# ma921/BASQ

Hardware: AMD Instinct MI355X
Metric: recombination batches/sec (N candidates -> n points) at N=1e6 d=10 (higher is better)
Workload: dtype f64

## Files before the change

basq_amd/_batch.py:

```python
from __future__ import annotations

import dataclasses
import time
import warnings

import torch

from . import _config as cfg
from . import _epochs
from ._basis import _mm_splitk, _ShardedProducts, _skip_test_matrix_draw, _Timer, make_cov_psd, nystrom_basis_steps
from ._lib import ROLE_A, ROLE_B
from ._partition import RoundGeometry, initial_shards
from ._plan import Plan, ReductionTimeout, _NoWait, _recorded_event, classes_for, late_split
from ._rounds_async import AsyncRounds
from ._rounds_sync import SyncRounds
from ._sums import FusedSums, OpaqueSums, exact_unit_plan


class Batch(AsyncRounds, SyncRounds):

    def __init__(self, ops, comm, pts_local, gid0: int, n_total: int, pts_nys, num_pts: int, kernel, trace=None,
                 variant: str = "basq", init_weights=None, objective=None, pipelined: bool = False, owner: int | None = None,
                 draw_on_owner: bool = False):
        if n_total >= 2 ** 31:
            raise ValueError("pool sizes >= 2^31 are not supported")
        self.ops, self.comm, self.trace = ops, comm, trace
        self.notes = []
        d = int(pts_nys.shape[1]) if pts_nys.dim() == 2 else 0
        if not getattr(kernel, "opaque", False) and not kernel.base.fits_packed_rows(d):
            from .kernels import CallableKernel

            self.notes.append(f"dimension {d} exceeds the fused kernels' packed-row limit ({kernel.base.__class__.__name__}: "
                              "d <= 38); the kernel is evaluated densely on the device (basq_dense_blocksum_f64 path)")
            kernel = CallableKernel(kernel)
        self.kernel, self.variant = kernel, variant
        self.pts_local_in, self.pts_nys_in = pts_local, pts_nys
        self.gid0, self.n_total, self.num_pts = int(gid0), int(n_total), int(num_pts)
        self.init_weights, self.objective = init_weights, objective
        self.pipelined = pipelined
        self.owner = None if (owner is None or comm.world == 1) else int(owner) % comm.world
        self.draw_on_owner = bool(draw_on_owner) and self.owner is not None
        m_nys = int(pts_nys.shape[0]) if pts_nys.dim() >= 1 else 0
        self.plan = Plan.of(kernel, variant, objective, comm, ops, trace, n_sets=2 * (min(int(num_pts) - 1, m_nys) + 1),
                            owner=self.owner)

    def steps(self):
        try:
            return (yield from self._steps())
        finally:
            self._release()

    def _release(self):
        sums = self.__dict__.get("sums")
        if sums is not None:
            sums.b = None
        keep = ("notes", "plan", "drew_test_matrix")
        for k in list(self.__dict__):
            if k not in keep:
                self.__dict__[k] = None

    def _steps(self):
        ops = self.ops
        if self.n_total == 0:
            dev = getattr(ops, "device", "cpu")
            return torch.empty(0, dtype=torch.int64, device=dev), torch.empty(0, dtype=torch.float64, device=dev)
        t_all = time.perf_counter()
        self._prepare_operands()
        self._init_candidates()
        pre, late = self._prelaunch_round1()
        t0 = time.perf_counter()
        U = yield from self._basis_steps(late)
        self._trace_phase("basis", t0)
        if self.trace is not None and self.trace.keep_tensors:
            self.trace.U = U.clone()
        self._extend_basis(U)
        self._trace_phase("setup", t0)
        if self.plan.async_rounds and self.R > self.S:
            if _epochs.eligible(self):
                outcome = yield from _epochs.async_rounds_columns(self, pre)
            else:
                outcome = yield from self._async_rounds(pre)
            pre = None
            if outcome == "basis":
                self._recover_basis()
                self._init_candidates()
            elif outcome:
                self.notes.append("descriptor-driven rounds hit a round that did not keep exactly half of the sets; the "
                                  "rounds were repeated one read-back at a time")
                self._init_candidates()
        if self._basis_bad is not None:
            flag, ready = ops.to_host_async(self._basis_bad, "basis_flag")
            yield ready
            if float(flag[0]) != 0.0:
                self._recover_basis()
            self._basis_bad = None
        idx, w = yield from self._sync_rounds(pre)
        self._trace_phase("total", t_all)
        for msg in self.notes:
            warnings.warn("basq_amd.recombination: " + msg, RuntimeWarning, stacklevel=3)
        return idx, w

    def _trace_phase(self, key, t0):
        if self.trace is not None:
            if self.trace.host_sync:
                self.ops.synchronize()
            self.trace.add_time(key, time.perf_counter() - t0)

    def _prepare_operands(self):
        ops, kernel, plan = self.ops, self.kernel, self.plan
        self.pts_nys = pts_nys = ops.to_device(self.pts_nys_in, torch.float64)
        self.pts_local = ops.to_device(self.pts_local_in, torch.float64)
        self.m, self.d = m, d = pts_nys.shape
        self.base = None if plan.opaque else kernel.base
        self.post = kernel.posterior if plan.posterior else None
        self.spec = None if plan.opaque else self.base.spec(d)
        if plan.posterior:
            self.spec = dataclasses.replace(self.spec, accurate_exp=True)
        self.kp = d if plan.opaque else ops.kp(d)
        self.kscale = 1.0 if plan.opaque else self.spec.outputscale
        self.center = None if plan.opaque else ops.col_mean(pts_nys)
# ... 26 lines not shown
            nys_cat = torch.cat(nys_rows, 0) if len(nys_rows) > 1 else pts_nys
            nys_ext = ops.pack(self.spec, nys_cat, self.center, ROLE_A, pad_rows_to=64)
            if nys_ext.shape[0] < ((self.m_ext + 63) // 64) * 64:
                nys_ext = torch.cat([nys_ext, ops.zeros(64, self.kp)], 0)
            if self.wrow:
                nys_ext[self.zero_row_idx].zero_()
            self.nys_ext = nys_ext
        self.exact_blocks = plan.opaque and kernel.resolve_mode(ops, pts_nys, self.S)
        self.sums = OpaqueSums(self) if plan.opaque else FusedSums(self)

    def _init_candidates(self):
        ops, comm, plan = self.ops, self.comm, self.plan
        pts_local = self.pts_local
        Rl = pts_local.shape[0]
        self.cand = (pts_local if Rl > 0 else ops.zeros(1, self.d)) if plan.opaque \
            else ops.pack(self.spec, pts_local, self.center, ROLE_B)
        self.mu, self.gid = ops.init_state(Rl, self.gid0, self.n_total)
        self.wx = None
        if plan.warp != "none":
            self.wx = self.kernel.mean(ops, pts_local, self.center) if Rl > 0 else ops.empty(1)
        self.off, self.R, self.Rl = self.gid0, self.n_total, Rl
        self.obj_full = self.obj_live = None
        if plan.objective:
            self.obj_full = self.obj_live = ops.to_device(self.objective, torch.float64).reshape(-1)
            if self.obj_full.shape[0] != Rl:
                raise ValueError("objective must have one entry per candidate")
        if plan.sober and self.init_weights is not None:
            w0 = ops.to_device(self.init_weights, torch.float64)
            if w0.shape[0] != Rl:
                raise ValueError("init_weights must have one entry per local candidate")
            nz = torch.nonzero(w0 != 0).reshape(-1)
            self.cand, self.mu, self.gid = self.cand[nz].contiguous(), w0[nz].contiguous(), self.gid[:Rl][nz].contiguous()
            if self.obj_live is not None:
                self.obj_live = self.obj_live[nz].contiguous()
            if self.wx is not None:
                self.wx = self.wx[nz].contiguous()
            Rl = int(nz.numel())
            counts = torch.tensor([float(Rl)], dtype=torch.float64, device=self.mu.device)
            if comm.world > 1:
                counts = comm.all_gather(counts).reshape(-1)
            counts = [int(v) for v in counts.cpu()]
            self.off, self.R, self.Rl = sum(counts[:comm.rank]), sum(counts), Rl
            if Rl == 0:
                self.cand, self.mu, self.gid = ops.zeros(1, self.kp), ops.zeros(1), ops.zeros(1, dtype=torch.int64)
        self.cls = None
        self.R_lo = self.R

    def _prelaunch_round1(self):
        if self.R > self.S and not self.plan.opaque:
            pre = self.sums.evaluate(RoundGeometry.of(self.R, self.S), self.S, defer_last=True)
            return pre, pre[5]
        return None, None

    def _basis_steps(self, late):
        ops, comm, kernel, trace = self.ops, self.comm, self.kernel, self.trace
        m, q, pts_nys = self.m, self.q, self.pts_nys
        self._basis_bad = self._basis_fallback = None
        self._basis_on_rank0 = False
        if cfg.SHARDED_BASIS and comm.world > 1 and not self.plan.sober and not self.plan.opaque:
            shards = initial_shards(m, comm.world)
            r0, mr = shards[comm.rank]
            with _Timer(ops, trace, "basis.gram"):
                A_rows = kernel.dense(ops, pts_nys[r0:r0 + mr].contiguous(), pts_nys, self.center, diag_offset=r0) \
                    if mr else ops.zeros(0, m)
            prod = _ShardedProducts(ops, comm, A_rows, shards, m, drawer=self.owner if self.draw_on_owner else 0,
                                    lockstep=not self.draw_on_owner)
            self.drew_test_matrix = comm.rank == prod.drawer or prod.lockstep
            res = yield from nystrom_basis_steps(ops, prod, self.num_pts - 1, trace, overlap=late, notes=self.notes)
            if res.bad is not None:
                self._basis_bad, self._basis_fallback = res.bad.to(torch.float64), res.fallback
            return res.U
        self._basis_on_rank0 = True
        bad = None
        if comm.rank == 0:
            with _Timer(ops, trace, "basis.gram"):
                A = kernel.dense(ops, pts_nys, pts_nys, self.center)
                if self.plan.sober:
                    A = make_cov_psd(A)
            res = yield from nystrom_basis_steps(ops, A, self.num_pts - 1, trace, overlap=late, notes=self.notes)
            del A
            U, bad, self._basis_fallback = res.U, res.bad, res.fallback
            assert U.shape[0] == q
        else:
            U = ops.empty(q, m)
            _skip_test_matrix_draw(ops, m, self.num_pts - 1)
            if late is not None:
                late()
            if cfg.BASIS_SVD and cfg.GPU_RANGE_FINDER and self.num_pts - 1 <= m:
                yield _recorded_event(ops)
        if comm.world > 1:
            buf = ops.empty(q + 1, m)
            if comm.rank == 0:
                buf[:q] = U
                buf[q].zero_()
                if bad is not None:
                    buf[q, 0:1] = bad.to(torch.float64)
            comm.broadcast(buf)
            U = buf[:q]
            self._basis_bad = buf[q, 0:1] if (cfg.GPU_RANGE_FINDER and not cfg.BASIS_SVD and self.num_pts - 1 <= m) else None
        elif bad is not None:
            self._basis_bad = bad.to(torch.float64)
        return U

    def _recover_basis(self):
        ops, comm = self.ops, self.comm
        if not self._basis_on_rank0:
            U = self._basis_fallback()
        else:
            U = self._basis_fallback() if comm.rank == 0 else ops.empty(self.q, self.m)
            if comm.world > 1:
                U = U.contiguous()
                comm.broadcast(U)
        if self.trace is not None and self.trace.keep_tensors:
            self.trace.U = U.clone()
        self._basis_bad = None
        self._extend_basis(U)

    def _extend_basis(self, U):
        ops, plan, q, m = self.ops, self.plan, self.q, self.m
        self.U = U
        Um = U
        if plan.warp != "none":
            mu_pt = self.kernel.mean(ops, self.pts_nys, self.center)
            Um = (U * mu_pt.unsqueeze(0)).contiguous()
        U_cols = [Um]
        self.bmatT = None
        if self.post is not None:
            W = ops.to_device(self.post.W, torch.float64)
            Bmat = _mm_splitk(ops, self.base.dense(ops, self.pts_nys, self.Xo, self.center), W, 1)
            U_cols.append(-_mm_splitk(ops, Um, Bmat, 8))
            if plan.warp == "wsabim":
                self.bmatT = ops.zeros(((self.n_obs + 3) // 4) * 4, ((m + 63) // 64) * 64)
                self.bmatT[:self.n_obs, :m] = Bmat.t()
        U_ext = torch.cat(U_cols, 1) if len(U_cols) > 1 else Um
# ... 7 lines not shown
```

basq_amd/_config.py:

```python
from __future__ import annotations

HOST_LAPACK_THREADS = 8
HOST_SVD_THREADS = 1

OWN_RANGE_GEMM = True
FUSED_CHOLQR = True
BASIS_SVD = False
GPU_RANGE_FINDER = True
GPU_NULLSPACE = True

REPLICATED_REDUCTION = True
OWNER_RANK_REDUCTION = True
SHARDED_CHOLQR = True
SHARDED_BASIS = True

LATE_CHUNKS = 0
LATE_CLASSES = 0
LATE_CLASSES_PIPELINED = 0

CLASS_SUMS = True
MAX_CLASSES = 16
IRR_COLUMNS = True
PIPELINED_SIDE_STREAM = False
ASYNC_ROUNDS = True

RAND_COPY_STREAM = True

SPIN_WAIT = False

PSD_EIG_MAX_M = 4096
```

basq_amd/_ops.py:

```python
from __future__ import annotations

import ctypes as C

import torch

from . import _lib
from ._lib import KernelSpecC, ROLE_A, ROLE_B, check


def _ptr(t):
    return C.c_void_p(t.data_ptr()) if t is not None else C.c_void_p(0)


_COPY_STREAMS = {}
_SIDE_OPS = {}
PROJECT_KSPLIT_MAX = 64


class HipOps:

    name = "hip"

    def __init__(self, device, stream=None):
        self.device = torch.device(device)
# ... 449 lines not shown
            W = torch.linalg.solve_triangular(torch.tril(G).t(), eye, upper=True)
            return torch.nan_to_num(W).contiguous(), info
        W = self.empty(q, q)
        check(self.lib.basq_chol_inv_f64(_ptr(G), q, _ptr(W), _ptr(info), float(rel_tol), self._stream()),
              "basq_chol_inv_f64")
        return W, info

    CHOL_FACTOR_MAX_Q = 200
    TRSM_MAX_Q = 318

    def chol_factor(self, G, rel_tol=1e-12):
        self._chk(G)
        info = self.empty(1, dtype=torch.int32)
        check(self.lib.basq_chol_factor_f64(_ptr(G), G.shape[0], _ptr(info), float(rel_tol), self._stream()),
              "basq_chol_factor_f64")
        return info

    def trsm_rows(self, X, L):
        self._chk(X)
        self._chk(L)
        rows, q = X.shape
        out = self.empty(rows, q)
        check(self.lib.basq_trsm_rows_f64(_ptr(X), q, rows, q, _ptr(L), _ptr(out), q, self._stream()), "basq_trsm_rows_f64")
        return out

    CHOLQR_FUSED_MAX_Q = 200

    def cholqr(self, G, X, rel_tol=1e-12):
        self._chk(G)
        self._chk(X)
        rows, q = X.shape
        out = self.empty(rows, q)
        info = self.empty(2, dtype=torch.int32)
        check(self.lib.basq_cholqr_f64(_ptr(G), q, _ptr(info), float(rel_tol), _ptr(X), q, rows, _ptr(out), q, self._stream()),
              "basq_cholqr_f64")
        return out, info[:1]

    def gemm(self, A, B, alpha=1.0):
        self._chk(A)
        self._chk(B)
        Mr, K = A.shape
        K2, N = B.shape
        assert K == K2
        Cm = self.empty(Mr, N)
        check(self.lib.basq_gemm_f64(_ptr(A), K, _ptr(B), N, _ptr(Cm), N, Mr, N, K, float(alpha), self._stream()),
              "basq_gemm_f64")
        return Cm

    def matmul(self, A, B):
        return torch.matmul(A, B)

    SKINNY_MAX_N = 208

    @staticmethod
    def _skinny_ksplit(M, K, N):
        rows_per_wave = 16 if N > 112 else 32
        row_waves = (M + rows_per_wave - 1) // rows_per_wave
        return max(1, min(round(1900 / row_waves), K // 160))

    def skinny_gemm(self, A, B, trans=False, ksplit=None):
        if A.dtype != torch.float64 or B.dtype != torch.float64 or A.stride(1) != 1 or B.stride(1) != 1:
            raise ValueError("expected float64 matrices with unit column stride")
        K, M = (A.shape[0], A.shape[1]) if trans else (A.shape[1], A.shape[0])
        N = B.shape[1]
        assert B.shape[0] == K and N <= self.SKINNY_MAX_N
        if ksplit is None:
            ksplit = self._skinny_ksplit(M, K, N)
        out = self.empty(M, N)
        work = self.empty(ksplit * M * N) if ksplit > 1 else None
        check(self.lib.basq_skinny_gemm_f64(_ptr(A), A.stride(0), 1 if trans else 0, M, K, _ptr(B), B.stride(0), N,
                                            int(ksplit), _ptr(work), _ptr(out), self._stream()), "basq_skinny_gemm_f64")
        return out

    PIN_CACHE_ENTRIES = 48

    def _pinned(self, shape, dtype, tag):
        cache = self.__dict__.setdefault("_pin_cache", {})
        key = (tag, tuple(shape), dtype)
        buf = cache.pop(key, None)
        if buf is None:
            buf = torch.empty(tuple(shape), dtype=dtype, pin_memory=True)
            while len(cache) >= self.PIN_CACHE_ENTRIES:
                cache.pop(next(iter(cache)))
        cache[key] = buf
        return buf

    def release_caches(self):
        for k in ("_pin_cache", "_ws_cache", "_ut_cache"):
            self.__dict__.pop(k, None)

    def to_host(self, t, tag="d2h"):
        buf = self._pinned(t.shape, t.dtype, tag)
        buf.copy_(t, non_blocking=True)
        self.torch_stream().synchronize()
        return buf

    def to_host_async(self, t, tag="d2h"):
        buf = self._pinned(t.shape, t.dtype, tag)
        buf.copy_(t, non_blocking=True)
        ev = torch.cuda.Event()
        ev.record(self.torch_stream())
        return buf, ev

    def host_uniform(self, n, tag):
        buf = self._pinned((n,), torch.float64, tag)
        return torch.rand(n, dtype=torch.float64, out=buf)

    def from_pinned(self, buf):
        return buf.to(self.device, non_blocking=True)

    def from_pinned_side(self, buf):
        side = _COPY_STREAMS.get(self.device.index)
        if side is None:
            side = _COPY_STREAMS[self.device.index] = torch.cuda.Stream(device=self.device)
        with torch.cuda.stream(side):
            t = buf.to(self.device, non_blocking=True)
            ev = torch.cuda.Event()
            ev.record(side)
        main = self.torch_stream()
        main.wait_event(ev)
        t.record_stream(main)
        return t

    def from_host(self, t, tag="h2d"):
        buf = self._pinned(t.shape, t.dtype, tag)
        buf.copy_(t)
        return buf.to(self.device, non_blocking=True)

    def synchronize(self):
        self.torch_stream().synchronize()

    def record_event(self, timing=True):
        ev = torch.cuda.Event(enable_timing=timing)
        ev.record(self.torch_stream())
        return ev

    def wait_event(self, ev):
        self.torch_stream().wait_event(ev)

    def side_ops(self):
        idx = self.device.index
        ops = _SIDE_OPS.get(idx)
        if ops is None:
            ops = _SIDE_OPS[idx] = HipOps(self.device, stream=torch.cuda.Stream(device=self.device))
        return ops

    def own_side_ops(self):
        ops = self.__dict__.get("_own_side")
        if ops is None:
            ops = self.__dict__["_own_side"] = HipOps(self.device, stream=torch.cuda.Stream(device=self.device))
        return ops

    def side_context(self):
        return torch.cuda.stream(self.side_ops().stream)

    def own_side_context(self):
        return torch.cuda.stream(self.own_side_ops().stream)
```

basq_amd/csrc/basq_linalg.hip:

```cpp
#include "basq_common.hpp"

template <int JT>
__global__ void __launch_bounds__(256) gemm_kernel(const double* __restrict__ A, long long lda, long long a_ks,
                                                   const double* __restrict__ B, long long ldb, long long bstride,
                                                   int nsum, double* __restrict__ C, long long ldc, long long cstride,
                                                   int M, int N, int K, int kslice, double alpha, int zdiv,
                                                   long long b_zstride) {
    const int lane = threadIdx.x & 63, wave = threadIdx.x >> 6;
    const int c = lane & 15, g = lane >> 4;
    const int r0 = blockIdx.x * (16 * JT);
    const int n0 = (blockIdx.y * 4 + wave) * 16;
    if (n0 >= N) return;
    B += (long long)(blockIdx.z / zdiv) * b_zstride;
    const int k0 = (blockIdx.z % zdiv) * kslice;
    int k1 = k0 + kslice;
    if (k1 > K) k1 = K;
    const int col = (n0 + c < N) ? (n0 + c) : (N - 1);
    long long arow[JT];
#pragma unroll
    for (int jt = 0; jt < JT; ++jt) {
        int r = r0 + jt * 16 + c;
        if (r >= M) r = M - 1;
        arow[jt] = (long long)r * lda;
    }
    d4 acc[JT];
#pragma unroll
    for (int jt = 0; jt < JT; ++jt) acc[jt] = (d4){0.0, 0.0, 0.0, 0.0};
    for (int k = k0; k < k1; k += 16) {
        double bv[4], av[4][JT];
#pragma unroll
        for (int u = 0; u < 4; ++u) {
            const int kg = k + 4 * u + g;
            const bool kin = kg < k1;
            double b = 0.0;
            if (kin) {
                const double* bp = B + (long long)kg * ldb + col;
                b = bp[0];
                for (int v = 1; v < nsum; ++v) b += bp[(long long)v * bstride];
            }
            bv[u] = b;
#pragma unroll
            for (int jt = 0; jt < JT; ++jt) av[u][jt] = kin ? A[arow[jt] + kg * a_ks] : 0.0;
        }
#pragma unroll
        for (int u = 0; u < 4; ++u)
#pragma unroll
            for (int jt = 0; jt < JT; ++jt)
                acc[jt] = __builtin_amdgcn_mfma_f64_16x16x4f64(av[u][jt], bv[u], acc[jt], 0, 0, 0);
    }
    if (n0 + c < N) {
        double* Cz = C + (long long)blockIdx.z * cstride;
#pragma unroll
        for (int jt = 0; jt < JT; ++jt)
#pragma unroll
            for (int r = 0; r < 4; ++r) {
                const int row = r0 + jt * 16 + g + 4 * r;
                if (row < M) Cz[(long long)row * ldc + n0 + c] = alpha * acc[jt][r];
            }
    }
}

template <int CTRL>
__device__ __forceinline__ double dpp_row_f64(double v) {
    const long long b = __double_as_longlong(v);
    const int lo = __builtin_amdgcn_mov_dpp((int)b, CTRL, 0xf, 0xf, true);
    const int hi = __builtin_amdgcn_mov_dpp((int)(b >> 32), CTRL, 0xf, 0xf, true);
    return __longlong_as_double(((long long)hi << 32) | (unsigned int)lo);
}

template <int NT, int REM, int JT, bool TRANS>
__global__ void __launch_bounds__(256) __attribute__((amdgpu_waves_per_eu(2)))
skinny_gemm_kernel(const double* __restrict__ A, long long lda, long long a_bstride, const double* __restrict__ B,
                   long long ldb, double* __restrict__ C, long long ldc, long long cstride, int M, int N, int K, int kslice,
                   int nz) {
    const int lane = threadIdx.x & 63, wave = threadIdx.x >> 6;
    const int c = lane & 15, g = lane >> 4;
    A += (long long)blockIdx.y * a_bstride;
    C += (long long)blockIdx.y * nz * cstride;
    const int zslice = blockIdx.x % nz;
    const int r0 = ((blockIdx.x / nz) * 4 + wave) * (16 * JT);
    const int k0 = zslice * kslice;
    int k1 = k0 + kslice;
    if (k1 > K) k1 = K;
    int rg[4];
    rg[0] = c >> 2;
    rg[1] = (__builtin_amdgcn_update_dpp(0, c, 0x124, 0xf, 0xf, false) & 15) >> 2;
    rg[2] = (__builtin_amdgcn_update_dpp(0, c, 0x128, 0xf, 0xf, false) & 15) >> 2;
    rg[3] = (__builtin_amdgcn_update_dpp(0, c, 0x12c, 0xf, 0xf, false) & 15) >> 2;
    long long aoff[JT];
#pragma unroll
    for (int jt = 0; jt < JT; ++jt) {
        int r = r0 + jt * 16 + c;
        if (r >= M) r = M - 1;
        aoff[jt] = TRANS ? (long long)r : (long long)r * lda;
    }
    constexpr int NB = NT + REM;
    constexpr int W = 16 * NT + 4 * REM;
    int bcol[NB];
#pragma unroll
    for (int nt = 0; nt < NT; ++nt) bcol[nt] = (nt * 16 + c < N) ? (nt * 16 + c) : (N - 1);
#pragma unroll
    for (int r = 0; r < REM; ++r) bcol[NT + r] = (16 * NT + 4 * r + (c & 3) < N) ? (16 * NT + 4 * r + (c & 3)) : (N - 1);
    double acc[JT][4][NT], accr[JT][REM > 0 ? REM : 1];
#pragma unroll
    for (int jt = 0; jt < JT; ++jt)
#pragma unroll
        for (int r = 0; r < (REM > 0 ? REM : 1); ++r) accr[jt][r] = 0.0;
#pragma unroll
    for (int jt = 0; jt < JT; ++jt)
#pragma unroll
        for (int rho = 0; rho < 4; ++rho)
#pragma unroll
            for (int nt = 0; nt < NT; ++nt) acc[jt][rho][nt] = 0.0;
    auto kidx = [&](int k, int u) { return TRANS ? (k + 4 * u + g) : (k + 4 * g + u); };
    const bool a_vec = !TRANS && ((lda & 1) == 0) && (((uintptr_t)A & 15) == 0);
    auto mfma_step = [&](const double (&a)[JT], const double (&bv)[NB]) {
#pragma unroll
        for (int jt = 0; jt < JT; ++jt) {
            double ar[4];
            ar[0] = a[jt];
            ar[1] = dpp_row_f64<0x124>(ar[0]);
            ar[2] = dpp_row_f64<0x128>(ar[0]);
            ar[3] = dpp_row_f64<0x12c>(ar[0]);
#pragma unroll
            for (int rho = 0; rho < 4; ++rho)
#pragma unroll
                for (int nt = 0; nt < NT; ++nt)
                    acc[jt][rho][nt] = __builtin_amdgcn_mfma_f64_4x4x4f64(ar[rho], bv[nt], acc[jt][rho][nt], 0, 0, 0);
#pragma unroll
            for (int r = 0; r < REM; ++r)
                accr[jt][r] = __builtin_amdgcn_mfma_f64_4x4x4f64(a[jt], bv[NT + r], accr[jt][r], 0, 0, 0);
        }
    };

    constexpr int NLD = (W + 15) / 16;
    __shared__ double btile[2][16][W];
    const int over_rows = (W + (int)ldb - 1) / (int)ldb;
    const int kfast_end = (k1 < K - over_rows) ? k1 : (K - over_rows);
    const int ktrips = (kfast_end > k0) ? (kfast_end - k0) / 16 : 0;
    int kdone = k0;
    if (ktrips > 0 && (TRANS || a_vec)) {
        const int skk = threadIdx.x >> 4, sc = threadIdx.x & 15;
        const char* bbase = reinterpret_cast<const char*>(B + (long long)k0 * ldb);
        const unsigned soff = (unsigned)(((long long)skk * ldb + sc) * 8);
        const long long btrip = 16 * ldb * 8;
        auto stage_load = [&](double (&sr)[NLD]) {
#pragma unroll
            for (int i = 0; i < NLD; ++i)
                if (16 * i + 16 <= W || sc + 16 * i < W) sr[i] = *reinterpret_cast<const double*>(bbase + soff + 128 * i);
        };
        auto stage_store = [&](int buf, const double (&sr)[NLD]) {
#pragma unroll
            for (int i = 0; i < NLD; ++i)
                if (16 * i + 16 <= W || sc + 16 * i < W) btile[buf][skk][sc + 16 * i] = sr[i];
        };
        auto lds_b = [&](int buf, int u, double (&bv)[NB]) {
            const int kk = TRANS ? (4 * u + g) : (4 * g + u);
#pragma unroll
            for (int nt = 0; nt < NT; ++nt) bv[nt] = btile[buf][kk][16 * nt + c];
#pragma unroll
            for (int r = 0; r < REM; ++r) bv[NT + r] = btile[buf][kk][16 * NT + 4 * r + (c & 3)];
        };
        const double* ap[JT];
#pragma unroll
        for (int jt = 0; jt < JT; ++jt) ap[jt] = TRANS ? (A + (long long)(k0 + g) * lda + aoff[jt]) : (A + aoff[jt] + k0 + 4 * g);
        const long long atrip = TRANS ? 16 * lda : 16;
        auto fetch_a = [&](double (&av)[4][JT]) {
#pragma unroll
            for (int jt = 0; jt < JT; ++jt) {
                if (TRANS) {
#pragma unroll
                    for (int u = 0; u < 4; ++u) av[u][jt] = ap[jt][(long long)(4 * u) * lda];
                } else {
                    const double2* p = reinterpret_cast<const double2*>(ap[jt]);
                    const double2 lo = p[0], hi = p[1];
                    av[0][jt] = lo.x;
                    av[1][jt] = lo.y;
                    av[2][jt] = hi.x;
                    av[3][jt] = hi.y;
                }
            }
        };
        double av[4][JT], bv[NB], sr[NLD];
        fetch_a(av);
        stage_load(sr);
        stage_store(0, sr);
        __syncthreads();
        lds_b(0, 0, bv);
        for (int t = 0; t < ktrips; ++t) {
            const bool last = (t + 1 == ktrips);
            const int buf = t & 1;
            if (!last) {
                bbase += btrip;
                stage_load(sr);
            }
            const long long ainc = last ? 0 : atrip;
#pragma unroll
            for (int jt = 0; jt < JT; ++jt) ap[jt] += ainc;
            double avn[4][JT];
            fetch_a(avn);
#pragma unroll
            for (int u = 0; u < 4; ++u) {
                double bvn[NB];
                if (u < 3) lds_b(buf, u + 1, bvn);
                mfma_step(av[u], bv);
                if (u < 3) {
#pragma unroll
                    for (int nt = 0; nt < NB; ++nt) bv[nt] = bvn[nt];
                }
            }
            if (!last) stage_store(buf ^ 1, sr);
            __syncthreads();
            if (!last) lds_b(buf ^ 1, 0, bv);
#pragma unroll
            for (int u = 0; u < 4; ++u)
#pragma unroll
                for (int jt = 0; jt < JT; ++jt) av[u][jt] = avn[u][jt];
        }
        kdone = k0 + 16 * ktrips;
    }
    for (int k = kdone; k < k1; k += 16) {
#pragma unroll
        for (int u = 0; u < 4; ++u) {
            const int kk = kidx(k, u);
            const int kc = (kk < k1) ? kk : (k1 - 1);
            double a[JT], bv[NB];
#pragma unroll
            for (int jt = 0; jt < JT; ++jt) {
                const double v = TRANS ? A[(long long)kc * lda + aoff[jt]] : A[aoff[jt] + kc];
                a[jt] = (kk < k1) ? v : 0.0;
            }
            const double* bp = B + (long long)kc * ldb;
#pragma unroll
            for (int nt = 0; nt < NB; ++nt) bv[nt] = bp[bcol[nt]];
            mfma_step(a, bv);
        }
    }
    double* Cz = C + (long long)zslice * cstride;
#pragma unroll
    for (int nt = 0; nt < NT; ++nt) {
        if (nt * 16 + c >= N) continue;
#pragma unroll
        for (int jt = 0; jt < JT; ++jt)
#pragma unroll
            for (int rho = 0; rho < 4; ++rho) {
                const int row = r0 + jt * 16 + 4 * rg[rho] + g;
                if (row < M) Cz[(long long)row * ldc + nt * 16 + c] = acc[jt][rho][nt];
            }
    }
#pragma unroll
    for (int r = 0; r < REM; ++r) {
        const int col = 16 * NT + 4 * r + (c & 3);
        if (col >= N) continue;
#pragma unroll
        for (int jt = 0; jt < JT; ++jt) {
            const int row = r0 + jt * 16 + 4 * (c >> 2) + g;
            if (row < M) Cz[(long long)row * ldc + col] = accr[jt][r];
        }
    }
}

template <int NT, int REM, int JT>
static void launch_skinny(bool trans, int M, int nz, int nbatch, hipStream_t st, const double* A, long long lda,
                          long long a_bstride, const double* B, long long ldb, double* C, long long ldc, long long cstride,
                          int N, int K, int kslice) {
    dim3 grid((unsigned)((M + 64 * JT - 1) / (64 * JT)) * (unsigned)nz, (unsigned)nbatch);
    if (trans)
        hipLaunchKernelGGL((skinny_gemm_kernel<NT, REM, JT, true>), grid, dim3(256), 0, st, A, lda, a_bstride, B, ldb, C, ldc,
                           cstride, M, N, K, kslice, nz);
    else
        hipLaunchKernelGGL((skinny_gemm_kernel<NT, REM, JT, false>), grid, dim3(256), 0, st, A, lda, a_bstride, B, ldb, C, ldc,
                           cstride, M, N, K, kslice, nz);
}

static void dispatch_skinny(bool trans, int M, int nz, int nbatch, hipStream_t st, const double* A, long long lda,
                            long long a_bstride, const double* B, long long ldb, double* C, long long cstride, int N, int K,
                            int kslice) {
    const int nt = (N + 15) / 16, ng = (N + 3) / 4;
    const bool small = (long long)((M + 127) / 128) * nz * nbatch <= 128;
    if (small && ng == 25) launch_skinny<6, 1, 1>(trans, M, nz, nbatch, st, A, lda, a_bstride, B, ldb, C, N, cstride, N, K, kslice);
    else if (small && nt <= 4) launch_skinny<4, 0, 1>(trans, M, nz, nbatch, st, A, lda, a_bstride, B, ldb, C, N, cstride, N, K, kslice);
    else if (small && nt <= 7) launch_skinny<7, 0, 1>(trans, M, nz, nbatch, st, A, lda, a_bstride, B, ldb, C, N, cstride, N, K, kslice);
    else if (ng == 25) launch_skinny<6, 1, 2>(trans, M, nz, nbatch, st, A, lda, a_bstride, B, ldb, C, N, cstride, N, K, kslice);
    else if (ng == 50) launch_skinny<12, 2, 1>(trans, M, nz, nbatch, st, A, lda, a_bstride, B, ldb, C, N, cstride, N, K, kslice);
    else if (nt <= 4) launch_skinny<4, 0, 2>(trans, M, nz, nbatch, st, A, lda, a_bstride, B, ldb, C, N, cstride, N, K, kslice);
    else if (nt <= 7) launch_skinny<7, 0, 2>(trans, M, nz, nbatch, st, A, lda, a_bstride, B, ldb, C, N, cstride, N, K, kslice);
    else launch_skinny<13, 0, 1>(trans, M, nz, nbatch, st, A, lda, a_bstride, B, ldb, C, N, cstride, N, K, kslice);
}

__global__ void chunk_sum_kernel(const double* __restrict__ Xpart, long long n, int n_chunks, double* __restrict__ Xsum) {
    const long long e = ((long long)blockIdx.x * blockDim.x + threadIdx.x) * 2;
    if (e + 1 < n) {
        double2 v = *reinterpret_cast<const double2*>(Xpart + e);
        for (int c = 1; c < n_chunks; ++c) {
            const double2 u = *reinterpret_cast<const double2*>(Xpart + (long long)c * n + e);
            v.x += u.x;
            v.y += u.y;
        }
        *reinterpret_cast<double2*>(Xsum + e) = v;
    } else if (e < n) {
        double v = Xpart[e];
        for (int c = 1; c < n_chunks; ++c) v += Xpart[(long long)c * n + e];
        Xsum[e] = v;
    }
}

__device__ __forceinline__ double ordered_strided_sum(const double* __restrict__ p, int n, long long stride) {
    double v = 0.0;
    int z = 0;
    for (; z + 8 <= n; z += 8) {
        double t[8];
#pragma unroll
        for (int u = 0; u < 8; ++u) t[u] = p[(long long)(z + u) * stride];
#pragma unroll
        for (int u = 0; u < 8; ++u) v += t[u];
    }
    for (; z < n; ++z) v += p[(long long)z * stride];
    return v;
}

__global__ void project_reduce_kernel(const double* __restrict__ work, int ksplit, int q, int S,
                                      const double* __restrict__ totpart, int n_chunks, double* __restrict__ out) {
    const int idx = blockIdx.x * blockDim.x + threadIdx.x;
    if (idx >= (q + 1) * S) return;
    const int r = idx / S, s = idx % S;
    double v = 0.0;
    if (r == 0) {
        for (int cc = 0; cc < n_chunks; ++cc) v += totpart[(long long)cc * S + s];
    } else {
        v = ordered_strided_sum(work + (long long)(r - 1) * S + s, ksplit, (long long)q * S);
    }
    out[idx] = v;
}

__global__ void finalize_kernel(const double* __restrict__ parts, int n_parts, int msg_rows, int q, int S,
                                const double* __restrict__ diagU, long long ld_diag, int n_diag, double diag_noise,
                                int diag_wrow, int diag_tail_row, int n_tail_diag, double* __restrict__ XcarT,
                                double* __restrict__ tot_out, const long long* __restrict__ geo) {
    const int idx = blockIdx.x * blockDim.x + threadIdx.x;
    if (idx >= (q + 1) * S) return;
// ... 773 lines not shown
    if (idx >= per * n_chunks) return;
    const int c = (int)(idx / per);
    const int e = (int)(idx - (long long)c * per);
    const int r = e / S, s2 = e - r * S;
    double v = 0.0;
    if (r == 0) {
        v = totpart[(long long)c * S + s2];
    } else {
        v = ordered_strided_sum(work + ((long long)c * nz * q + (r - 1)) * S + s2, nz, (long long)q * S);
    }
    out[idx] = v;
}

__global__ void project_chunks_reduce_t_kernel(const double* __restrict__ work, int nz, int q, int S,
                                               const double* __restrict__ totpart, int n_chunks, double outputscale,
                                               double* __restrict__ out) {
    const long long idx = (long long)blockIdx.x * blockDim.x + threadIdx.x;
    const long long per = (long long)(q + 1) * S;
    if (idx >= per * n_chunks) return;
    const int c = (int)(idx / per);
    const int e = (int)(idx - (long long)c * per);
    const int s2 = e / (q + 1), r = e - s2 * (q + 1);
    double v = 0.0;
    if (r == 0) {
        v = totpart[(long long)c * S + s2];
    } else {
        v = outputscale * ordered_strided_sum(work + ((long long)c * nz * S + s2) * q + (r - 1), nz, (long long)S * q);
    }
    out[((long long)c * (q + 1) + r) * S + s2] = v;
}

__global__ void sum_parts_kernel(const double* __restrict__ parts, int n_parts, long long n, double* __restrict__ out) {
    const long long e = (long long)blockIdx.x * blockDim.x + threadIdx.x;
    if (e >= n) return;
    out[e] = ordered_strided_sum(parts + e, n_parts, n);
}

int basq_project_chunks_f64(const double* Ut, int32_t q, int32_t m, const double* Xpart, const double* totpart,
                            int32_t n_chunks, int32_t S, double outputscale, int32_t ksplit, double* work, double* out,
                            void* stream) {
    if (!Ut || !Xpart || !totpart || !work || !out || q < 1 || m < 1 || S < 1 || n_chunks < 1 || ksplit < 1)
        return BASQ_EINVAL;
    hipStream_t st = (hipStream_t)stream;
    if (q <= 208 && n_chunks <= 65535) {
        const int rows_per_wg = (q > 112) ? 64 : 128;
        const int rowblocks = (S + rows_per_wg - 1) / rows_per_wg;
        int want = 2048 / (rowblocks * n_chunks * 4);
        if (want > m / 64) want = m / 64;
        if (want > ksplit) want = ksplit;
        if (want < 1) want = 1;
        int kslice = (m + want - 1) / want;
        kslice = ((kslice + 15) / 16) * 16;
        const int nz = (m + kslice - 1) / kslice;
        dispatch_skinny(true, S, nz, n_chunks, st, Xpart, (long long)S, (long long)m * S, Ut, (long long)q, work,
                        (long long)S * q, q, m, kslice);
        BASQ_CHECK_LAUNCH();
        const long long tot = (long long)(q + 1) * S * n_chunks;
        hipLaunchKernelGGL(project_chunks_reduce_t_kernel, dim3((unsigned)((tot + 255) / 256)), dim3(256), 0, st, work, nz, q,
                           S, totpart, n_chunks, outputscale, out);
        BASQ_CHECK_LAUNCH();
        return BASQ_OK;
    }
    int kslice = (m + ksplit - 1) / ksplit;
    kslice = ((kslice + 15) / 16) * 16;
    const int nz = (m + kslice - 1) / kslice;
    if ((long long)n_chunks * nz > 65535) return BASQ_EINVAL;
    dim3 grid((unsigned)((q + 111) / 112), (unsigned)((S + 63) / 64), (unsigned)(n_chunks * nz));
    hipLaunchKernelGGL((gemm_kernel<7>), grid, dim3(256), 0, st, Ut, 1LL, (long long)q, Xpart, (long long)S, 0LL, 1, work,
                       (long long)S, (long long)q * S, q, S, m, kslice, outputscale, nz, (long long)m * S);
    BASQ_CHECK_LAUNCH();
    const long long tot = (long long)(q + 1) * S * n_chunks;
    hipLaunchKernelGGL(project_chunks_reduce_kernel, dim3((unsigned)((tot + 255) / 256)), dim3(256), 0, st, work, nz, q, S,
                       totpart, n_chunks, out);
    BASQ_CHECK_LAUNCH();
    return BASQ_OK;
}

int basq_sum_parts_f64(const double* parts, int32_t n_parts, int64_t n, double* out, void* stream) {
    if (!parts || !out || n_parts < 1 || n < 1) return BASQ_EINVAL;
    hipLaunchKernelGGL(sum_parts_kernel, dim3((unsigned)((n + 255) / 256)), dim3(256), 0, (hipStream_t)stream, parts, n_parts,
                       (long long)n, out);
    BASQ_CHECK_LAUNCH();
    return BASQ_OK;
}

int basq_finalize_geo_f64(const double* parts, int32_t n_parts, int32_t msg_rows, int32_t q, int32_t S,
                          const double* diagU, int64_t ld_diag, int32_t n_diag, double diag_noise, int32_t diag_wrow,
                          int32_t diag_tail_row, int32_t n_tail_diag, const int64_t* geo, double* XcarT, double* tot_out,
                          void* stream) {
    if (!parts || !XcarT || !tot_out || n_parts < 1 || q < 1 || S < 1 || msg_rows < q + 1) return BASQ_EINVAL;
    if (diag_wrow < 0 || diag_wrow >= msg_rows) return BASQ_EINVAL;
    if (diag_tail_row < 0 || diag_tail_row >= msg_rows || n_tail_diag < 0 || n_tail_diag > S) return BASQ_EINVAL;
    if (diagU && (n_diag > ld_diag || n_tail_diag > ld_diag)) return BASQ_EINVAL;
    const int tot = (q + 1) * S;
    hipLaunchKernelGGL(finalize_kernel, dim3((unsigned)((tot + 255) / 256)), dim3(256), 0, (hipStream_t)stream, parts,
                       n_parts, msg_rows, q, S, diagU, (long long)ld_diag, n_diag, diag_noise, diag_wrow, diag_tail_row,
                       n_tail_diag, XcarT, tot_out, (const long long*)geo);
    BASQ_CHECK_LAUNCH();
    return BASQ_OK;
}

int basq_finalize_f64(const double* parts, int32_t n_parts, int32_t msg_rows, int32_t q, int32_t S,
                      const double* diagU, int64_t ld_diag, int32_t n_diag, double diag_noise, int32_t diag_wrow,
                      int32_t diag_tail_row, int32_t n_tail_diag, double* XcarT, double* tot_out, void* stream) {
    return basq_finalize_geo_f64(parts, n_parts, msg_rows, q, S, diagU, ld_diag, n_diag, diag_noise, diag_wrow,
                                 diag_tail_row, n_tail_diag, nullptr, XcarT, tot_out, stream);
}

// ... 62 lines not shown
    if (lds > 163840 - 256) return BASQ_EUNSUPPORTED;
    const size_t lds_l = lds + (size_t)q * q * sizeof(double);
    const dim3 grid((unsigned)((rows + 63) / 64));
    if (lds_l <= 163840 - 256) {
        if (hipFuncSetAttribute((const void*)trsm_rows_kernel<true>, hipFuncAttributeMaxDynamicSharedMemorySize, (int)lds_l) !=
            hipSuccess)
            return BASQ_ELAUNCH;
        hipLaunchKernelGGL(trsm_rows_kernel<true>, grid, dim3(512), lds_l, (hipStream_t)stream, X, (long long)ldx,
                           (long long)rows, q, L, Q, (long long)ldq);
    } else {
        if (hipFuncSetAttribute((const void*)trsm_rows_kernel<false>, hipFuncAttributeMaxDynamicSharedMemorySize, (int)lds) !=
            hipSuccess)
            return BASQ_ELAUNCH;
        hipLaunchKernelGGL(trsm_rows_kernel<false>, grid, dim3(512), lds, (hipStream_t)stream, X, (long long)ldx,
                           (long long)rows, q, L, Q, (long long)ldq);
    }
    BASQ_CHECK_LAUNCH();
    return BASQ_OK;
}

int basq_cholqr_f64(double* G, int32_t q, int32_t* info, double rel_tol, const double* X, int64_t ldx, int64_t rows,
                    double* Q, int64_t ldq, void* stream) {
    if (!G || !info || !X || !Q || q < 1 || rows < 0 || ldx < q || ldq < q || !(rel_tol >= 0.0)) return BASQ_EINVAL;
    const size_t tri = (size_t)q * (q + 1) / 2 * sizeof(double);
    const size_t lds_full = ((size_t)64 * (q | 1) + (size_t)q * q) * sizeof(double);
    const size_t lds_rows = ((size_t)64 * (q | 1) + (size_t)BASQ_CHOL_NB * q) * sizeof(double);
    const bool full = lds_full <= 163840 - 512;
    const size_t lds = full ? lds_full : (lds_rows > tri ? lds_rows : tri);
    if (lds > 163840 - 512 || rows > 64LL * 4096) return BASQ_EUNSUPPORTED;
    hipStream_t st = (hipStream_t)stream;
    if (hipMemsetAsync(info, 0, 2 * sizeof(int32_t), st) != hipSuccess) return BASQ_ELAUNCH;
    const dim3 grid((unsigned)(1 + (rows + 63) / 64));
    if (full) {
        if (hipFuncSetAttribute((const void*)cholqr_fused_kernel<true>, hipFuncAttributeMaxDynamicSharedMemorySize, (int)lds) != hipSuccess)
            return BASQ_ELAUNCH;
        hipLaunchKernelGGL(cholqr_fused_kernel<true>, grid, dim3(512), lds, st, G, q, info, rel_tol, X, (long long)ldx,
                           (long long)rows, Q, (long long)ldq);
    } else {
        if (hipFuncSetAttribute((const void*)cholqr_fused_kernel<false>, hipFuncAttributeMaxDynamicSharedMemorySize, (int)lds) != hipSuccess)
            return BASQ_ELAUNCH;
        hipLaunchKernelGGL(cholqr_fused_kernel<false>, grid, dim3(512), lds, st, G, q, info, rel_tol, X, (long long)ldx,
                           (long long)rows, Q, (long long)ldq);
    }
    BASQ_CHECK_LAUNCH();
    return BASQ_OK;
}

int basq_skinny_gemm_f64(const double* A, int64_t lda, int32_t trans, int32_t M, int32_t K, const double* B, int64_t ldb,
                         int32_t N, int32_t ksplit, double* work, double* C, void* stream) {
    if (!A || !B || !C || M < 1 || N < 1 || K < 1 || ksplit < 1 || ldb < N) return BASQ_EINVAL;
    if (lda < (trans ? M : K)) return BASQ_EINVAL;
    if (N > 208 || ldb > (1LL << 24)) return BASQ_EUNSUPPORTED;
    hipStream_t st = (hipStream_t)stream;
    int kslice = (K + ksplit - 1) / ksplit;
    kslice = ((kslice + 15) / 16) * 16;
    const int nz = (K + kslice - 1) / kslice;
    if (nz > 1 && !work) return BASQ_EINVAL;
    double* out = (nz > 1) ? work : C;
    const long long cstride = (long long)M * N;
    dispatch_skinny(trans != 0, M, nz, 1, st, A, lda, 0LL, B, ldb, out, cstride, N, K, kslice);
    BASQ_CHECK_LAUNCH();
    if (nz > 1) {
        const long long n = cstride;
        hipLaunchKernelGGL(sum_parts_kernel, dim3((unsigned)((n + 255) / 256)), dim3(256), 0, st, work, nz, n, C);
        BASQ_CHECK_LAUNCH();
    }
    return BASQ_OK;
}

int basq_gemm_f64(const double* A, int64_t lda, const double* B, int64_t ldb, double* C, int64_t ldc, int32_t M,
                  int32_t N, int32_t K, double alpha, void* stream) {
    if (!A || !B || !C || M < 1 || N < 1 || K < 1 || lda < K || ldb < N || ldc < N) return BASQ_EINVAL;
    dim3 grid((unsigned)((M + 63) / 64), (unsigned)((N + 63) / 64), 1);
    const int kslice = ((K + 3) / 4) * 4;
    hipLaunchKernelGGL((gemm_kernel<4>), grid, dim3(256), 0, (hipStream_t)stream, A, (long long)lda, 1LL, B, (long long)ldb,
                       0LL, 1, C, (long long)ldc, 0LL, M, N, K, kslice, alpha, 1, 0LL);
    BASQ_CHECK_LAUNCH();
    return BASQ_OK;
}

}
```

Measured before the change: 60.36.

## Switch skinny GEMM to stream-K work split and optionally run range finder on side stream

Replaces the fixed split-K partitioning of the skinny f64 GEMM with a stream-K style scheme. Each workgroup processes a contiguous range of (row tile, k-step) units, sized to a resident-workgroup count derived from the CU count. Tiles split across workgroups write partial slabs that a new reduce kernel sums, while unsplit tiles write directly to the output. A flag-gated path (off by default) also runs the Nyström gram and range finder on a higher-priority side stream beside the round-1 sums. The aim is better load balance and fewer partial-sum passes, at the cost of more complex indexing, a persistent-loop kernel structure, and register pressure from the loop.

```diff
diff --git a/basq_amd/_batch.py b/basq_amd/_batch.py
--- a/basq_amd/_batch.py
+++ b/basq_amd/_batch.py
@@ -1,5 +1,6 @@
 from __future__ import annotations
 
+import contextlib
 import dataclasses
 import time
 import warnings
@@ -66,6 +67,7 @@
             return torch.empty(0, dtype=torch.int64, device=dev), torch.empty(0, dtype=torch.float64, device=dev)
         t_all = time.perf_counter()
         self._prepare_operands()
+        self._nys_ready = ops.record_event(False) if self._range_finder_beside_sums() else None
         self._init_candidates()
         pre, late = self._prelaunch_round1()
         t0 = time.perf_counter()
@@ -198,6 +200,11 @@
             return pre, pre[5]
         return None, None
 
+    def _range_finder_beside_sums(self):
+        return (cfg.RANGE_FINDER_BESIDE_SUMS and self.comm.world == 1 and not self.pipelined and not self.plan.opaque
+                and cfg.GPU_RANGE_FINDER and not cfg.BASIS_SVD and self.num_pts - 1 <= self.m
+                and hasattr(self.ops, "side_ops"))
+
     def _basis_steps(self, late):
         ops, comm, kernel, trace = self.ops, self.comm, self.kernel, self.trace
         m, q, pts_nys = self.m, self.q, self.pts_nys
@@ -219,13 +226,27 @@
         self._basis_on_rank0 = True
         bad = None
         if comm.rank == 0:
-            with _Timer(ops, trace, "basis.gram"):
-                A = kernel.dense(ops, pts_nys, pts_nys, self.center)
-                if self.plan.sober:
-                    A = make_cov_psd(A)
-            res = yield from nystrom_basis_steps(ops, A, self.num_pts - 1, trace, overlap=late, notes=self.notes)
-            del A
+            beside = self.__dict__.get("_nys_ready") is not None
+            rops = ops.side_ops() if beside else ops
+            if beside:
+                rops.wait_event(self._nys_ready)
+            with (ops.side_context() if beside else contextlib.nullcontext()):
+                with _Timer(rops, trace, "basis.gram"):
+                    A = kernel.dense(rops, pts_nys, pts_nys, self.center)
+                    if self.plan.sober:
+                        A = make_cov_psd(A)
+                res = yield from nystrom_basis_steps(rops, A, self.num_pts - 1, trace, overlap=None if beside else late,
+                                                     notes=self.notes)
+                del A
+                side_done = rops.record_event(False) if beside else None
             U, bad, self._basis_fallback = res.U, res.bad, res.fallback
+            if beside:
+                ops.wait_event(side_done)
+                for t in (U, bad):
+                    if t is not None:
+                        t.record_stream(ops.torch_stream())
+                if late is not None:
+                    late()
             assert U.shape[0] == q
         else:
             U = ops.empty(q, m)
diff --git a/basq_amd/_config.py b/basq_amd/_config.py
--- a/basq_amd/_config.py
+++ b/basq_amd/_config.py
@@ -18,6 +18,8 @@
 LATE_CLASSES = 0
 LATE_CLASSES_PIPELINED = 0
 
+RANGE_FINDER_BESIDE_SUMS = False
+
 CLASS_SUMS = True
 MAX_CLASSES = 16
 IRR_COLUMNS = True
diff --git a/basq_amd/_ops.py b/basq_amd/_ops.py
--- a/basq_amd/_ops.py
+++ b/basq_amd/_ops.py
@@ -525,11 +525,18 @@
 
     SKINNY_MAX_N = 208
 
-    @staticmethod
-    def _skinny_ksplit(M, K, N):
-        rows_per_wave = 16 if N > 112 else 32
-        row_waves = (M + rows_per_wave - 1) // rows_per_wave
-        return max(1, min(round(1900 / row_waves), K // 160))
+    SKINNY_RESIDENT_WGS = 512
+
+    @classmethod
+    def _skinny_ksplit(cls, M, K, N):
+        T = (K + 15) // 16
+        small = ((M + 127) // 128) * max(T // 10, 1) <= 128
+        rows = 64 if (small or N > 112) else 128
+        tiles = (M + rows - 1) // rows
+        units = tiles * T
+        wgs = max(1, min(cls.SKINNY_RESIDENT_WGS, units // 10))
+        upw = (units + wgs - 1) // wgs
+        return 1 if upw % T == 0 else (T + upw - 1) // upw + 1
 
     def skinny_gemm(self, A, B, trans=False, ksplit=None):
         if A.dtype != torch.float64 or B.dtype != torch.float64 or A.stride(1) != 1 or B.stride(1) != 1:
@@ -615,7 +622,10 @@
         idx = self.device.index
         ops = _SIDE_OPS.get(idx)
         if ops is None:
-            ops = _SIDE_OPS[idx] = HipOps(self.device, stream=torch.cuda.Stream(device=self.device))
+            from . import _config as cfg
+
+            prio = -1 if cfg.RANGE_FINDER_BESIDE_SUMS else 0
+            ops = _SIDE_OPS[idx] = HipOps(self.device, stream=torch.cuda.Stream(device=self.device, priority=prio))
         return ops
 
     def own_side_ops(self):
diff --git a/basq_amd/csrc/basq_linalg.hip b/basq_amd/csrc/basq_linalg.hip
--- a/basq_amd/csrc/basq_linalg.hip
+++ b/basq_amd/csrc/basq_linalg.hip
@@ -68,25 +68,36 @@
     return __longlong_as_double(((long long)hi << 32) | (unsigned int)lo);
 }
 
+__host__ __device__ constexpr bool skinny_one_segment(int NT, int REM, int JT) { return (4 * NT + REM) * JT > 50 || NT >= 12; }
+
 template <int NT, int REM, int JT, bool TRANS>
 __global__ void __launch_bounds__(256) __attribute__((amdgpu_waves_per_eu(2)))
 skinny_gemm_kernel(const double* __restrict__ A, long long lda, long long a_bstride, const double* __restrict__ B,
-                   long long ldb, double* __restrict__ C, long long ldc, long long cstride, int M, int N, int K, int kslice,
-                   int nz) {
+                   long long ldb, double* __restrict__ C1, double* __restrict__ Cs, long long ldc, long long cstride, int M,
+                   int N, int K, int T, int upw, int nslab, int ntiles) {
     const int lane = threadIdx.x & 63, wave = threadIdx.x >> 6;
     const int c = lane & 15, g = lane >> 4;
     A += (long long)blockIdx.y * a_bstride;
-    C += (long long)blockIdx.y * nz * cstride;
-    const int zslice = blockIdx.x % nz;
-    const int r0 = ((blockIdx.x / nz) * 4 + wave) * (16 * JT);
-    const int k0 = zslice * kslice;
-    int k1 = k0 + kslice;
+    C1 += (long long)blockIdx.y * nslab * cstride;
+    Cs += (long long)blockIdx.y * nslab * cstride;
+    constexpr int NB = NT + REM;
+    constexpr int W = 16 * NT + 4 * REM;
+    constexpr int NLD = (W + 15) / 16;
+    __shared__ double btile[2][16][W];
+    const int over_rows = (W + (int)ldb - 1) / (int)ldb;
+    const bool a_vec = !TRANS && ((lda & 1) == 0) && (((uintptr_t)A & 15) == 0);
+    int unit = (int)blockIdx.x * upw;
+    const int unit_end = (ntiles * T - unit < upw) ? ntiles * T : unit + upw;
+    constexpr bool ONE_SEGMENT = skinny_one_segment(NT, REM, JT);
+#pragma nounroll
+    while (unit < unit_end) {
+    const int tile = __builtin_amdgcn_readfirstlane(unit / T);
+    const int t0 = unit - tile * T;
+    const int t1 = (unit_end - tile * T < T) ? (unit_end - tile * T) : T;
+    const int r0 = (tile * 4 + wave) * (16 * JT);
+    int k1 = t1 * 16;
     if (k1 > K) k1 = K;
-    int rg[4];
-    rg[0] = c >> 2;
-    rg[1] = (__builtin_amdgcn_update_dpp(0, c, 0x124, 0xf, 0xf, false) & 15) >> 2;
-    rg[2] = (__builtin_amdgcn_update_dpp(0, c, 0x128, 0xf, 0xf, false) & 15) >> 2;
-    rg[3] = (__builtin_amdgcn_update_dpp(0, c, 0x12c, 0xf, 0xf, false) & 15) >> 2;
+    const int k0 = (t0 * 16 < k1) ? t0 * 16 : k1;
     long long aoff[JT];
 #pragma unroll
     for (int jt = 0; jt < JT; ++jt) {
@@ -94,13 +105,6 @@
         if (r >= M) r = M - 1;
         aoff[jt] = TRANS ? (long long)r : (long long)r * lda;
     }
-    constexpr int NB = NT + REM;
-    constexpr int W = 16 * NT + 4 * REM;
-    int bcol[NB];
-#pragma unroll
-    for (int nt = 0; nt < NT; ++nt) bcol[nt] = (nt * 16 + c < N) ? (nt * 16 + c) : (N - 1);
-#pragma unroll
-    for (int r = 0; r < REM; ++r) bcol[NT + r] = (16 * NT + 4 * r + (c & 3) < N) ? (16 * NT + 4 * r + (c & 3)) : (N - 1);
     double acc[JT][4][NT], accr[JT][REM > 0 ? REM : 1];
 #pragma unroll
     for (int jt = 0; jt < JT; ++jt)
@@ -113,7 +117,6 @@
 #pragma unroll
             for (int nt = 0; nt < NT; ++nt) acc[jt][rho][nt] = 0.0;
     auto kidx = [&](int k, int u) { return TRANS ? (k + 4 * u + g) : (k + 4 * g + u); };
-    const bool a_vec = !TRANS && ((lda & 1) == 0) && (((uintptr_t)A & 15) == 0);
     auto mfma_step = [&](const double (&a)[JT], const double (&bv)[NB]) {
 #pragma unroll
         for (int jt = 0; jt < JT; ++jt) {
@@ -133,9 +136,6 @@
         }
     };
 
-    constexpr int NLD = (W + 15) / 16;
-    __shared__ double btile[2][16][W];
-    const int over_rows = (W + (int)ldb - 1) / (int)ldb;
     const int kfast_end = (k1 < K - over_rows) ? k1 : (K - over_rows);
     const int ktrips = (kfast_end > k0) ? (kfast_end - k0) / 16 : 0;
     int kdone = k0;
@@ -220,6 +220,11 @@
         kdone = k0 + 16 * ktrips;
     }
     for (int k = kdone; k < k1; k += 16) {
+        int bcol[NB];
+#pragma unroll
+        for (int nt = 0; nt < NT; ++nt) bcol[nt] = (nt * 16 + c < N) ? (nt * 16 + c) : (N - 1);
+#pragma unroll
+        for (int r = 0; r < REM; ++r) bcol[NT + r] = (16 * NT + 4 * r + (c & 3) < N) ? (16 * NT + 4 * r + (c & 3)) : (N - 1);
 #pragma unroll
         for (int u = 0; u < 4; ++u) {
             const int kk = kidx(k, u);
@@ -236,7 +241,16 @@
             mfma_step(a, bv);
         }
     }
-    double* Cz = C + (long long)zslice * cstride;
+    const int tile_u0 = tile * T;
+    unit = tile_u0 + t1;
+    const int wg_first = __builtin_amdgcn_readfirstlane(tile_u0 / upw);
+    const int nseg = __builtin_amdgcn_readfirstlane((tile_u0 + T - 1) / upw) - wg_first + 1;
+    double* Cz = (nseg == 1) ? C1 : (Cs + (long long)((int)blockIdx.x - wg_first) * cstride);
+    int rg[4];
+    rg[0] = c >> 2;
+    rg[1] = (__builtin_amdgcn_update_dpp(0, c, 0x124, 0xf, 0xf, false) & 15) >> 2;
+    rg[2] = (__builtin_amdgcn_update_dpp(0, c, 0x128, 0xf, 0xf, false) & 15) >> 2;
+    rg[3] = (__builtin_amdgcn_update_dpp(0, c, 0x12c, 0xf, 0xf, false) & 15) >> 2;
 #pragma unroll
     for (int nt = 0; nt < NT; ++nt) {
         if (nt * 16 + c >= N) continue;
@@ -258,34 +272,78 @@
             if (row < M) Cz[(long long)row * ldc + col] = accr[jt][r];
         }
     }
-}
+    if (ONE_SEGMENT) break;
+    }
+}
+
+struct SkinnyLaunch {
+    int T, upw, grid, nslab;
+};
 
 template <int NT, int REM, int JT>
-static void launch_skinny(bool trans, int M, int nz, int nbatch, hipStream_t st, const double* A, long long lda,
-                          long long a_bstride, const double* B, long long ldb, double* C, long long ldc, long long cstride,
-                          int N, int K, int kslice) {
-    dim3 grid((unsigned)((M + 64 * JT - 1) / (64 * JT)) * (unsigned)nz, (unsigned)nbatch);
+static void launch_skinny(bool trans, int M, const SkinnyLaunch& L, int nbatch, hipStream_t st, const double* A, long long lda,
+                          long long a_bstride, const double* B, long long ldb, double* C1, double* Cs, long long ldc,
+                          long long cstride, int N, int K) {
+    const int ntiles = (M + 64 * JT - 1) / (64 * JT);
+    dim3 grid((unsigned)L.grid, (unsigned)nbatch);
     if (trans)
-        hipLaunchKernelGGL((skinny_gemm_kernel<NT, REM, JT, true>), grid, dim3(256), 0, st, A, lda, a_bstride, B, ldb, C, ldc,
-                           cstride, M, N, K, kslice, nz);
+        hipLaunchKernelGGL((skinny_gemm_kernel<NT, REM, JT, true>), grid, dim3(256), 0, st, A, lda, a_bstride, B, ldb, C1, Cs,
+                           ldc, cstride, M, N, K, L.T, L.upw, L.nslab, ntiles);
     else
-        hipLaunchKernelGGL((skinny_gemm_kernel<NT, REM, JT, false>), grid, dim3(256), 0, st, A, lda, a_bstride, B, ldb, C, ldc,
-                           cstride, M, N, K, kslice, nz);
-}
-
-static void dispatch_skinny(bool trans, int M, int nz, int nbatch, hipStream_t st, const double* A, long long lda,
-                            long long a_bstride, const double* B, long long ldb, double* C, long long cstride, int N, int K,
-                            int kslice) {
+        hipLaunchKernelGGL((skinny_gemm_kernel<NT, REM, JT, false>), grid, dim3(256), 0, st, A, lda, a_bstride, B, ldb, C1, Cs,
+                           ldc, cstride, M, N, K, L.T, L.upw, L.nslab, ntiles);
+}
+
+static int skinny_rows_per_wg(int N, bool small) {
     const int nt = (N + 15) / 16, ng = (N + 3) / 4;
-    const bool small = (long long)((M + 127) / 128) * nz * nbatch <= 128;
-    if (small && ng == 25) launch_skinny<6, 1, 1>(trans, M, nz, nbatch, st, A, lda, a_bstride, B, ldb, C, N, cstride, N, K, kslice);
-    else if (small && nt <= 4) launch_skinny<4, 0, 1>(trans, M, nz, nbatch, st, A, lda, a_bstride, B, ldb, C, N, cstride, N, K, kslice);
-    else if (small && nt <= 7) launch_skinny<7, 0, 1>(trans, M, nz, nbatch, st, A, lda, a_bstride, B, ldb, C, N, cstride, N, K, kslice);
-    else if (ng == 25) launch_skinny<6, 1, 2>(trans, M, nz, nbatch, st, A, lda, a_bstride, B, ldb, C, N, cstride, N, K, kslice);
-    else if (ng == 50) launch_skinny<12, 2, 1>(trans, M, nz, nbatch, st, A, lda, a_bstride, B, ldb, C, N, cstride, N, K, kslice);
-    else if (nt <= 4) launch_skinny<4, 0, 2>(trans, M, nz, nbatch, st, A, lda, a_bstride, B, ldb, C, N, cstride, N, K, kslice);
-    else if (nt <= 7) launch_skinny<7, 0, 2>(trans, M, nz, nbatch, st, A, lda, a_bstride, B, ldb, C, N, cstride, N, K, kslice);
-    else launch_skinny<13, 0, 1>(trans, M, nz, nbatch, st, A, lda, a_bstride, B, ldb, C, N, cstride, N, K, kslice);
+    if (small && (ng == 25 || nt <= 7)) return 64;
+    if (ng == 25) return 128;
+    if (ng == 50) return 64;
+    return (nt <= 7) ? 128 : 64;
+}
+
+static bool skinny_single_segment(int N, bool small) {
+    const int nt = (N + 15) / 16, ng = (N + 3) / 4;
+    if ((small && nt <= 7) || ng == 25) return false;
+    return ng == 50 || nt > 4;
+}
+
+static void dispatch_skinny(bool trans, bool small, int M, const SkinnyLaunch& L, int nbatch, hipStream_t st, const double* A,
+                            long long lda, long long a_bstride, const double* B, long long ldb, double* C1, double* Cs,
+                            long long cstride, int N, int K) {
+    const int nt = (N + 15) / 16, ng = (N + 3) / 4;
+    if (small && ng == 25) launch_skinny<6, 1, 1>(trans, M, L, nbatch, st, A, lda, a_bstride, B, ldb, C1, Cs, N, cstride, N, K);
+    else if (small && nt <= 4) launch_skinny<4, 0, 1>(trans, M, L, nbatch, st, A, lda, a_bstride, B, ldb, C1, Cs, N, cstride, N, K);
+    else if (small && nt <= 7) launch_skinny<7, 0, 1>(trans, M, L, nbatch, st, A, lda, a_bstride, B, ldb, C1, Cs, N, cstride, N, K);
+    else if (ng == 25) launch_skinny<6, 1, 2>(trans, M, L, nbatch, st, A, lda, a_bstride, B, ldb, C1, Cs, N, cstride, N, K);
+    else if (ng == 50) launch_skinny<12, 2, 1>(trans, M, L, nbatch, st, A, lda, a_bstride, B, ldb, C1, Cs, N, cstride, N, K);
+    else if (nt <= 4) launch_skinny<4, 0, 2>(trans, M, L, nbatch, st, A, lda, a_bstride, B, ldb, C1, Cs, N, cstride, N, K);
+    else if (nt <= 7) launch_skinny<7, 0, 2>(trans, M, L, nbatch, st, A, lda, a_bstride, B, ldb, C1, Cs, N, cstride, N, K);
+    else launch_skinny<13, 0, 1>(trans, M, L, nbatch, st, A, lda, a_bstride, B, ldb, C1, Cs, N, cstride, N, K);
+}
+
+static int skinny_resident_wgs() {
+    static int n = 0;
+    if (n == 0) {
+        int dev = 0, cu = 0;
+        if (hipGetDevice(&dev) != hipSuccess || hipDeviceGetAttribute(&cu, hipDeviceAttributeMultiprocessorCount, dev) != hipSuccess ||
+            cu < 1)
+            cu = 256;
+        n = 2 * cu;
+    }
+    return n;
+}
+
+__global__ void streamk_reduce_kernel(const double* __restrict__ slabs, long long n, int N, int rows_per_tile, int T, int upw,
+                                      double* __restrict__ C) {
+    const long long e = (long long)blockIdx.x * blockDim.x + threadIdx.x;
+    if (e >= n) return;
+    const int tile_u0 = (int)(e / N / rows_per_tile) * T;
+    const int nseg = (tile_u0 + T - 1) / upw - tile_u0 / upw + 1;
+    if (nseg == 1) return;
+    double v = 0.0;
+    for (int z = 0; z < nseg; ++z) v += slabs[(long long)z * n + e];
+    C[e] = v;
 }
 
 __global__ void chunk_sum_kernel(const double* __restrict__ Xpart, long long n, int n_chunks, double* __restrict__ Xsum) {
@@ -1165,8 +1223,11 @@
         int kslice = (m + want - 1) / want;
         kslice = ((kslice + 15) / 16) * 16;
         const int nz = (m + kslice - 1) / kslice;
-        dispatch_skinny(true, S, nz, n_chunks, st, Xpart, (long long)S, (long long)m * S, Ut, (long long)q, work,
-                        (long long)S * q, q, m, kslice);
+        const bool small = (long long)((S + 127) / 128) * nz * n_chunks <= 128;
+        const int rows = skinny_rows_per_wg(q, small);
+        const SkinnyLaunch L = {nz * (kslice / 16), kslice / 16, ((S + rows - 1) / rows) * nz, nz};
+        dispatch_skinny(true, small, S, L, n_chunks, st, Xpart, (long long)S, (long long)m * S, Ut, (long long)q, work, work,
+                        (long long)S * q, q, m);
         BASQ_CHECK_LAUNCH();
         const long long tot = (long long)(q + 1) * S * n_chunks;
         hipLaunchKernelGGL(project_chunks_reduce_t_kernel, dim3((unsigned)((tot + 255) / 256)), dim3(256), 0, st, work, nz, q,
@@ -1335,17 +1396,37 @@
     if (lda < (trans ? M : K)) return BASQ_EINVAL;
     if (N > 208 || ldb > (1LL << 24)) return BASQ_EUNSUPPORTED;
     hipStream_t st = (hipStream_t)stream;
-    int kslice = (K + ksplit - 1) / ksplit;
-    kslice = ((kslice + 15) / 16) * 16;
-    const int nz = (K + kslice - 1) / kslice;
-    if (nz > 1 && !work) return BASQ_EINVAL;
-    double* out = (nz > 1) ? work : C;
+    const int T = (K + 15) / 16;
+    const bool small = (long long)((M + 127) / 128) * (T >= 10 ? T / 10 : 1) <= 128;
+    const int rows = skinny_rows_per_wg(N, small);
+    const long long ntiles = (M + rows - 1) / rows;
+    const long long units = ntiles * T;
+    long long wgs = units / 10;
+    if (wgs > skinny_resident_wgs()) wgs = skinny_resident_wgs();
+    if (wgs < 1) wgs = 1;
+    long long upw = (units + wgs - 1) / wgs;
+    const int cap = work ? ksplit : 1;
+    if (cap == 1) {
+        upw = (long long)T * ((ntiles + wgs - 1) / wgs);
+    } else if ((T + upw - 1) / upw + 1 > cap && upw % T != 0) {
+        const long long need = (T + cap - 2) / (cap - 1);
+        if (upw < need) upw = need;
+    }
+    int Tl = T;
+    if (skinny_single_segment(N, small)) {
+        const long long p = (T + upw - 1) / upw;
+        upw = (T + p - 1) / p;
+        Tl = (int)(p * upw);
+    }
+    const long long units_l = ntiles * Tl;
+    if (units_l + upw > 0x7fffffffLL) return BASQ_EUNSUPPORTED;
     const long long cstride = (long long)M * N;
-    dispatch_skinny(trans != 0, M, nz, 1, st, A, lda, 0LL, B, ldb, out, cstride, N, K, kslice);
+    const SkinnyLaunch L = {Tl, (int)upw, (int)((units_l + upw - 1) / upw), 1};
+    dispatch_skinny(trans != 0, small, M, L, 1, st, A, lda, 0LL, B, ldb, C, work ? work : C, cstride, N, K);
     BASQ_CHECK_LAUNCH();
-    if (nz > 1) {
-        const long long n = cstride;
-        hipLaunchKernelGGL(sum_parts_kernel, dim3((unsigned)((n + 255) / 256)), dim3(256), 0, st, work, nz, n, C);
+    if (upw % Tl != 0) {
+        hipLaunchKernelGGL(streamk_reduce_kernel, dim3((unsigned)((cstride + 255) / 256)), dim3(256), 0, st, work, cstride, N,
+                           rows, Tl, (int)upw, C);
         BASQ_CHECK_LAUNCH();
     }
     return BASQ_OK;
```

Result: no change. 60.06 (-0.5%).
